# nayuki/DEFLATE-library-Java

Measured on AMD Instinct MI355X. Metric: input MiB/s (compress+decompress), higher is better.
Workload: dtype u8

## Files before the change

### deflate-library-java_amd/csrc/capi/ndfl_deflate_batch_chunked.cpp

```cpp

struct SegTables {
    std::vector<SegChunk> chunks;
    std::vector<SegStream> streams;
    uint64_t staged = 0;
    uint64_t out_bytes = 0;
    bool any_sum = false;
};

static uint64_t seg_out_slot(uint64_t len, uint32_t chunk_len) {
    return ((ndfl_deflate_bound(len, chunk_len) + 8 + 3) / 4 + 2) * 4;
}

static int seg_build_tables(const ndfl_member_item* items, uint32_t n, uint32_t chunk_len, SegTables& T) {
    uint64_t nch = 0;
    for (uint32_t i = 0; i < n; i++) {
        const uint64_t len = items[i].in_len;
        nch += len == 0 ? 1 : len / chunk_len + (len % chunk_len != 0);
        if (nch > 0xFFFFFFFFull) return NDFL_E_UNSUPPORTED;
    }
    T.chunks.resize(nch);
    T.streams.resize(n);
    T.staged = nch * chunk_len;
    T.any_sum = false;
    uint64_t k = 0, obase = 0;
    for (uint32_t i = 0; i < n; i++) {
        const ndfl_member_item& it = items[i];
        const uint64_t len = it.in_len;
        const uint32_t cnt = (uint32_t)(len == 0 ? 1 : len / chunk_len + (len % chunk_len != 0));
        const uint32_t kind = it.format == NDFL_FMT_ZLIB ? NDFL_SUM_ADLER32 : it.format == NDFL_FMT_GZIP ? NDFL_SUM_CRC32 : it.sum;
        T.any_sum = T.any_sum || kind != NDFL_SUM_NONE;
        T.streams[i] = SegStream{obase, (uint32_t)k, cnt};
        obase += seg_out_slot(len, chunk_len);
        for (uint32_t j = 0; j < cnt; j++) {
            const uint64_t at = (uint64_t)j * chunk_len;
            SegChunk& c = T.chunks[k + j];
            c.start = k * chunk_len;
            c.src = it.in_off + at;
            c.stream = i;
            c.len = (uint32_t)std::min<uint64_t>(chunk_len, len - at);
            c.flags = (j == 0 ? SEG_FIRST : 0u) | (j + 1 == cnt ? SEG_LAST : 0u) | kind << SEG_SUM_SHIFT;
            c.pad = 0;
        }
        k += cnt;
    }
    T.out_bytes = obase;
    return NDFL_OK;
}

static int seg_launch_rle(ndfl_ctx* c, hipStream_t s, const SegTab tab, const uint8_t* slots, uint32_t nch, uint64_t staged,
                          uint32_t chunk_len, uint32_t hist_limit, int rle, int dyn) {
    HIPCHK(c->d_hist.ensure((size_t)nch * HREC * 4));
    HIPCHK(c->d_codes.ensure((size_t)nch * CREC * 4));
    const uint32_t ntile = (nch + SCAN_TILE - 1) / SCAN_TILE;
    HIPCHK(c->d_off.ensure(((size_t)2 * nch + 8 + ntile) * 8));
    uint64_t* d_offs = c->d_off.as<uint64_t>();
    uint64_t* d_raw = d_offs + nch;
    uint64_t* d_total = d_raw + nch;
    uint64_t* d_part = d_total + 8;
    Args a;
    a.in = slots; a.n = staged; a.chunk_len = chunk_len; a.nchunks = nch;
    a.prev_byte = -1; a.hist_enabled = hist_limit > 0; a.final_last = 1;
    a.rle = rle; a.dynamic = dyn; a.base_bit = 0; a.parent_len = chunk_len;
    a.out = c->d_out.as<uint32_t>(); a.status = c->d_status.as<uint64_t>(); a.ticket = c->d_ticket.as<uint32_t>();
    a.edge_w = c->d_edge_w.as<uint64_t>(); a.edge_v = c->d_edge_v.as<uint32_t>();
    a.chunk_bits = nullptr; a.crc_raw = nullptr;
    a.crc_tab = c->d_tabs.as<uint32_t>(); a.crc_x = c->d_tabs.as<uint32_t>() + 1024;
    a.prof = nullptr;
    a.hist_out = c->d_hist.as<uint32_t>(); a.codes = c->d_codes.as<uint32_t>(); a.chunk_off = d_offs;
    a.c0 = 0;
    a.pf_dist = c->knobs.deflate_pf ? 2u * (uint32_t)c->ncu : 0u;
    hipLaunchKernelGGL(ndfl_deflate_hist_seg_kernel, dim3(nch), dim3(1024), 0, s, a, tab);
    HIPCHK(hipGetLastError());
    hipLaunchKernelGGL(ndfl_deflate_codes_seg_kernel, dim3(nch), dim3(64), 0, s, a, tab);
    HIPCHK(hipGetLastError());
    hipLaunchKernelGGL(ndfl_deflate_offsets_sum_kernel, dim3(ntile), dim3(SCAN_T), 0, s, (const uint64_t*)a.status, nch, d_part);
    HIPCHK(hipGetLastError());
    hipLaunchKernelGGL(ndfl_deflate_offsets_kernel, dim3(ntile), dim3(SCAN_T), 0, s, (const uint64_t*)a.status, nch,
                       (uint64_t)0, d_raw, d_total, (const uint64_t*)d_part);
    HIPCHK(hipGetLastError());
    hipLaunchKernelGGL(ndfl_deflate_offsets_seg_kernel, dim3((nch + 255) / 256), dim3(256), 0, s, (const uint64_t*)d_raw,
                       a.status, nch, tab, d_offs);
    HIPCHK(hipGetLastError());
    hipLaunchKernelGGL(ndfl_deflate_emit_seg_kernel, dim3(nch), dim3(1024), 0, s, a, tab);
    HIPCHK(hipGetLastError());
    return NDFL_OK;
}

static int seg_launch_lz(ndfl_ctx* c, hipStream_t s, const SegTab tab, const uint8_t* buf, uint32_t nch, uint64_t staged,
                         uint32_t chunk_len, uint32_t hist_limit, const LzTuple& t, int dyn) {
    const uint64_t total = LZ_DS + staged;
    const uint32_t slab_ch = (uint32_t)std::min<uint64_t>(nch, std::max<uint64_t>(1, c->knobs.seg_slab / chunk_len));
    HIPCHK(c->d_match.ensure((size_t)slab_ch * chunk_len * 4));
    LzArgs la;
    la.buf = buf; la.total = total; la.vstart = LZ_DS; la.chunk_len = chunk_len; la.parent_len = chunk_len;
    la.hist_limit = hist_limit; la.min_run = (uint32_t)t.min_run; la.max_run = (uint32_t)t.max_run;
    la.min_dist = (uint32_t)t.min_dist; la.max_dist = (uint32_t)t.max_dist;
    la.link = nullptr; la.L0 = 0; la.match = c->d_match.as<uint32_t>(); la.stats = nullptr;
    LzEncArgs ea;
    ea.match = c->d_match.as<uint32_t>(); ea.n = staged; ea.chunk_len = chunk_len; ea.nchunks = nch;
    ea.final_last = 1; ea.dynamic = dyn; ea.base_bit = 0;
    ea.out = c->d_out.as<uint32_t>(); ea.status = c->d_status.as<uint64_t>(); ea.ticket = c->d_ticket.as<uint32_t>();
    ea.edge_w = c->d_edge_w.as<uint64_t>(); ea.edge_v = c->d_edge_v.as<uint32_t>();
    ea.chunk_bits = nullptr; ea.match_rw = c->d_match.as<uint32_t>();
// ... 33 lines not shown
    SegTab tab;
    tab.chunks = c->d_segtab.as<SegChunk>();
    tab.streams = (const SegStream*)((char*)c->d_segtab.p + chunks_b);

    HIPCHK(c->d_lz.ensure(LZ_DS + T.staged + 64));
    uint8_t* buf = c->d_lz.as<uint8_t>();
    uint8_t* slots = buf + LZ_DS;
    HIPCHK(hipMemsetAsync(buf, 0, LZ_DS, s));
    HIPCHK(hipMemsetAsync(slots + T.staged, 0, 64, s));
    std::unique_ptr<uint8_t[]> pack;
    if (flags & NDFL_IN_DEVICE) {
        hipLaunchKernelGGL(ndfl_seg_gather_kernel, dim3(nch), dim3(256), 0, s, in, slots, tab, chunk_len);
        HIPCHK(hipGetLastError());
    } else {
        pack.reset(new (std::nothrow) uint8_t[T.staged]);
        if (!pack) return NDFL_E_INTERNAL;
        for (uint32_t k = 0; k < nch; k++) {
            const SegChunk& ch = T.chunks[k];
            uint8_t* dst = pack.get() + (uint64_t)k * chunk_len;
            if (ch.len) memcpy(dst, in + ch.src, ch.len);
            if (ch.len < chunk_len) memset(dst + ch.len, 0, chunk_len - ch.len);
        }
        HIPCHK(hipMemcpyAsync(slots, pack.get(), T.staged, hipMemcpyHostToDevice, s));
    }

    HIPCHK(c->d_out.ensure(T.out_bytes));
    HIPCHK(c->d_status.ensure(nch * sizeof(uint64_t)));
    HIPCHK(c->d_ticket.ensure(64));
    HIPCHK(c->d_edge_w.ensure(2ull * nch * sizeof(uint64_t)));
    HIPCHK(c->d_edge_v.ensure(2ull * nch * sizeof(uint32_t)));
    HIPCHK(c->d_crc.ensure(2ull * nch * sizeof(uint32_t)));
    HIPCHK(c->d_crc1.ensure(std::max<size_t>(64, (size_t)n * sizeof(uint32_t))));
    const int preset = lz77_preset(t, dynamic);

    auto launch = [&](hipStream_t q, uint8_t* d_out, const ndfl_member_item* d_items, ndfl_deflate_result* d_res,
                      uint32_t*) -> int {
        HIPCHK(hipMemsetAsync(c->d_status.p, 0, nch * sizeof(uint64_t), q));
        if (preset >= 0)
            TRY(seg_launch_rle(c, q, tab, slots, nch, T.staged, chunk_len, hist_limit,
                               preset == NDFL_RLE_STATIC || preset == NDFL_RLE_DYNAMIC, dynamic != 0));
        else
            TRY(seg_launch_lz(c, q, tab, buf, nch, T.staged, chunk_len, hist_limit, t, dynamic != 0));
        const uint32_t ne = 2 * nch;
        hipLaunchKernelGGL(ndfl_edge_fixup_kernel, dim3((ne + 255) / 256), dim3(256), 0, q, (const uint64_t*)c->d_edge_w.p,
                           (const uint32_t*)c->d_edge_v.p, ne, c->d_out.as<uint32_t>());
        HIPCHK(hipGetLastError());
        uint32_t* d_sums = c->d_crc1.as<uint32_t>();
        if (T.any_sum) {
            hipLaunchKernelGGL(ndfl_seg_sums_kernel, dim3(nch), dim3(1024), 0, q, (const uint8_t*)slots, chunk_len, tab,
                               (const uint32_t*)c->d_tabs.as<uint32_t>(), (const uint32_t*)(c->d_tabs.as<uint32_t>() + 1024),
                               c->d_crc.as<uint32_t>());
            HIPCHK(hipGetLastError());
            hipLaunchKernelGGL(ndfl_seg_sums_combine_kernel, dim3((uint32_t)(((uint64_t)n * 64 + 255) / 256)), dim3(256), 0, q,
                               (const uint32_t*)c->d_crc.p, chunk_len, tab, d_items, n,
                               (const uint32_t*)(c->d_tabs.as<uint32_t>() + 1024 + 64 + 1024), d_sums);
            HIPCHK(hipGetLastError());
        } else {
            HIPCHK(hipMemsetAsync(d_sums, 0, (size_t)n * sizeof(uint32_t), q));
        }
        hipLaunchKernelGGL(ndfl_seg_finish_kernel, dim3(n), dim3(1024), 0, q, c->d_out.as<uint8_t>(),
                           (const uint64_t*)c->d_status.p, tab, d_items, (const uint32_t*)d_sums, d_out, d_res);
        return NDFL_OK;
    };
    return batch_status(batch_run(c->batch, s, c->ev0, c->ev1, out, items, results, n, flags, &c->last_ms, launch));
}

extern "C" int ndfl_deflate_batch_chunked(ndfl_ctx* c, const uint8_t* in, uint64_t in_size, uint8_t* out, uint64_t out_size,
                                          const ndfl_member_item* items, ndfl_deflate_result* results, uint32_t n,
                                          int dynamic, int min_run, int max_run, int min_dist, int max_dist,
                                          uint32_t chunk_len, uint32_t hist_limit, uint32_t flags) {
    if (!c) return NDFL_E_ARG;
    if (n == 0) return NDFL_OK;
    const LzTuple t{min_run, max_run, min_dist, max_dist};
    if (!lz77_tuple_valid(t)) return NDFL_E_ARG;
    if (const int e = deflate_batch_args(in, in_size, out, out_size, items, results, n, chunk_len, hist_limit)) return e;
    return deflate_batch_chunked_run(c, in, out, items, results, n, t, dynamic, chunk_len, hist_limit, flags);
}
```

### deflate-library-java_amd/csrc/capi/ndfl_deflate_chunks.cpp

```cpp
#define TRY(x) do { if (const int _rc = (x)) return _rc; } while (0)

struct LzTuple {
    int min_run, max_run, min_dist, max_dist;
    bool literal_only() const { return min_run == 0 && max_run == 0 && min_dist == 0 && max_dist == 0; }
};
static LzTuple desc_tuple(const ndfl_strategy_desc& d) { return LzTuple{d.min_run, d.max_run, d.min_dist, d.max_dist}; }

static bool lz77_tuple_valid(const LzTuple& t) {
    const int min_run = t.min_run, max_run = t.max_run, min_dist = t.min_dist, max_dist = t.max_dist;
    return t.literal_only() || (3 <= min_run && min_run <= max_run && max_run <= 258 && 1 <= min_dist &&
                                min_dist <= max_dist && max_dist <= 32768);
}

static int lz77_preset(const LzTuple& t, int dynamic) {
    if (t.literal_only()) return dynamic ? NDFL_LITERAL_DYNAMIC : NDFL_LITERAL_STATIC;
    if (t.min_run == 3 && t.max_run == 258 && t.min_dist == 1 && t.max_dist == 1)
        return dynamic ? NDFL_RLE_DYNAMIC : NDFL_RLE_STATIC;
    return -1;
}

struct BlockOpts {
    uint64_t* chunk_bits = nullptr;
    uint32_t parent_len = 0;
};
// ... 106 lines not shown
    HIPCHK(hipMemsetAsync(c->d_ticket.p, 0, 64, s));

    Args a;
    a.in = d_data; a.n = f.len; a.chunk_len = f.chunk_len; a.nchunks = nch;
    a.prev_byte = prev_byte; a.hist_enabled = f.hist_limit > 0; a.final_last = f.final_flag ? 1 : 0;
    a.rle = rle; a.dynamic = dyn; a.base_bit = f.start_bitpos;
    a.parent_len = o.parent_len ? o.parent_len : f.chunk_len;
    a.out = f.d_out; a.status = c->d_status.as<uint64_t>(); a.ticket = c->d_ticket.as<uint32_t>();
    a.edge_w = c->d_edge_w.as<uint64_t>(); a.edge_v = c->d_edge_v.as<uint32_t>();
    a.chunk_bits = o.chunk_bits;
    a.crc_raw = f.crc_inout ? c->d_crc.as<uint32_t>() : nullptr;
    a.crc_tab = c->d_tabs.as<uint32_t>();
    a.crc_x = c->d_tabs.as<uint32_t>() + 1024;
    ScopedBuf prof;
    if (c->knobs.deflate_profile) {
        HIPCHK(prof.ensure((size_t)nch * 64));
        HIPCHK(hipMemsetAsync(prof.p, 0, (size_t)nch * 64, s));
    }
    a.prof = prof.as<uint64_t>();
    a.hist_out = nullptr; a.codes = nullptr; a.chunk_off = nullptr;
    a.pf_dist = c->knobs.deflate_pf ? 2u * (uint32_t)c->ncu : 0u;
    const bool split = !c->knobs.deflate_fused && !prof.p;
    uint64_t* d_total = nullptr;
    if (split) {
        HIPCHK(c->d_hist.ensure((size_t)nch * HREC * 4));
        HIPCHK(c->d_codes.ensure((size_t)nch * CREC * 4));
        HIPCHK(c->d_off.ensure((size_t)nch * 8 + 64 + (size_t)((nch + SCAN_TILE - 1) / SCAN_TILE) * 8));
        a.hist_out = c->d_hist.as<uint32_t>();
        a.codes = c->d_codes.as<uint32_t>();
        a.chunk_off = c->d_off.as<uint64_t>();
        d_total = c->d_off.as<uint64_t>() + nch;
    }
    a.c0 = 0;
    TRY(f.start_timing());
    if (split) {
        hipLaunchKernelGGL(ndfl_deflate_hist_kernel, dim3(nch), dim3(1024), 0, s, a);
        HIPCHK(hipGetLastError());
        hipLaunchKernelGGL(ndfl_deflate_codes_kernel, dim3(nch), dim3(64), 0, s, a);
        HIPCHK(hipGetLastError());
        const uint32_t ntile = (nch + SCAN_TILE - 1) / SCAN_TILE;
        uint64_t* d_part = c->d_off.as<uint64_t>() + nch + 8;
        hipLaunchKernelGGL(ndfl_deflate_offsets_sum_kernel, dim3(ntile), dim3(SCAN_T), 0, s, (const uint64_t*)a.status,
                           nch, d_part);
        HIPCHK(hipGetLastError());
        hipLaunchKernelGGL(ndfl_deflate_offsets_kernel, dim3(ntile), dim3(SCAN_T), 0, s, (const uint64_t*)a.status, nch,
                           (uint64_t)f.start_bitpos, c->d_off.as<uint64_t>(), d_total, (const uint64_t*)d_part);
        HIPCHK(hipGetLastError());
        hipLaunchKernelGGL(ndfl_deflate_emit_kernel, dim3(nch), dim3(1024), 0, s, a);
    } else {
        hipLaunchKernelGGL(ndfl_deflate_chunks_kernel, dim3(nch), dim3(1024), 0, s, a);
    }
    HIPCHK(hipGetLastError());
    TRY(f.stop_timing());
    const uint32_t ne = 2 * nch;
    hipLaunchKernelGGL(ndfl_edge_fixup_kernel, dim3((ne + 255) / 256), dim3(256), 0, s,
                       (const uint64_t*)a.edge_w, (const uint32_t*)a.edge_v, ne, f.d_out);
    HIPCHK(hipGetLastError());
    if (f.crc_inout) {
        HIPCHK(launch_crc_combine(c, s, (const uint32_t*)a.crc_raw, nch, f.chunk_len, f.len, c->d_crc1.as<uint32_t>()));
        HIPCHK(hipMemcpyAsync(c->h_pinned + 4, c->d_crc1.p, 4, hipMemcpyDeviceToHost, s));
    }
    TRY(f.read_end(split ? d_total : a.status + (nch - 1)));
    if (prof.p) {
        std::vector<uint64_t> h((size_t)nch * 8);
        HIPCHK(hipMemcpy(h.data(), prof.p, (size_t)nch * 64, hipMemcpyDeviceToHost));
        double sum[7] = {0}, tmin = 1e300, tmax = 0;
        for (uint32_t k = 0; k < nch; k++) {
            const uint64_t* q = &h[k * 8];
            for (int p = 0; p < 7; p++) sum[p] += (double)(q[p + 1] - q[p]);
            tmin = std::min(tmin, (double)q[0]); tmax = std::max(tmax, (double)q[7]);
        }
        fprintf(stderr, "[ndfl] deflate phases (us/chunk): load+crc %.2f hist %.2f codes %.2f bits+scan %.2f emit %.2f "
                "lookback %.2f store %.2f; span %.2f ms\n", sum[0] / nch / 100, sum[1] / nch / 100, sum[2] / nch / 100,
                sum[3] / nch / 100, sum[4] / nch / 100, sum[5] / nch / 100, sum[6] / nch / 100, (tmax - tmin) / 1e5);
    }
    if (f.crc_inout) {
        uint32_t raw = c->h_pinned[4];
        uint32_t dc = ~(crc_multmodp(crc_x8n(f.len), 0xFFFFFFFFu) ^ raw);
        *f.crc_inout = ndfl_crc32_combine(*f.crc_inout, dc, f.len);
    }
    return f.finish();
}

static int chunks_lz(Frame& f, const LzTuple& t, int dyn, BlockOpts o) {
    ndfl_ctx* c = f.c;
    hipStream_t s = f.s;
    const uint32_t nch = f.nch, chunk_len = f.chunk_len;
    const uint64_t len = f.len;
    const uint64_t total = LZ_DS + len;
    HIPCHK(c->d_lz.ensure(total + 64));
    uint8_t* buf = c->d_lz.as<uint8_t>();
    const hipMemcpyKind kin = (f.flags & NDFL_IN_DEVICE) ? hipMemcpyDeviceToDevice : hipMemcpyHostToDevice;
    if (f.hist_len) HIPCHK(hipMemcpyAsync(buf + LZ_DS - f.hist_len, f.hist, f.hist_len, kin, s));
    if (len) HIPCHK(hipMemcpyAsync(buf + LZ_DS, f.data, len, kin, s));
    HIPCHK(hipMemsetAsync(buf + total, 0, 64, s));
// ... 408 lines not shown
```

### deflate-library-java_amd/csrc/hip/deflate_kernels.hip

```cpp
#pragma once
#include "huffman_build.hpp"
#include "seg_tables.hpp"

namespace {

constexpr int DT = 1024;
constexpr int NW = DT / 64;
constexpr int MAX_CHUNK = 65536;
constexpr int OUTW = 18600;
static_assert(sizeof(HuffScr) <= OUTW * 4, "the code-construction scratch is laid over the bit buffer");

constexpr uint64_t ST_AGG = 1ull << 62;
constexpr uint64_t ST_PRE = 2ull << 62;
constexpr uint64_t ST_VAL = (1ull << 62) - 1;

struct Persist {
    uint32_t litCode[288];
    uint32_t distCode[32];
    uint64_t scan64[NW];
    uint32_t scan32[NW];
    uint32_t chunk;
    uint32_t hdrBits;
    uint64_t P;
    uint32_t crcAcc[NW];
};

struct Args {
    const uint8_t* in;
    uint64_t n;
    uint32_t chunk_len;
    uint32_t nchunks;
    int32_t prev_byte;
    int32_t hist_enabled;
    int32_t final_last;
    int32_t rle;
    int32_t dynamic;
    uint32_t parent_len;
    uint32_t base_bit;
    uint32_t* out;
    uint64_t* status;
    uint32_t* ticket;
    uint64_t* edge_w;
    uint32_t* edge_v;
    uint64_t* chunk_bits;
    uint32_t* crc_raw;
    const uint32_t* crc_tab;
    const uint32_t* crc_x;
    uint64_t* prof;
    uint32_t* hist_out;
    const uint32_t* codes;
    const uint64_t* chunk_off;
    uint32_t c0;
    uint32_t pf_dist;
};

constexpr int HREC = 320;
constexpr int CREC_LIT = 0;
constexpr int CREC_DIST = 288;
constexpr int CREC_HDR = 320;
constexpr int CREC_META = CREC_HDR + HDRW;
constexpr int CREC = CREC_META + 16;
enum { MODE_FUSED = 0, MODE_HIST = 1, MODE_EMIT = 2 };
#ifndef NDFL_HCOPY
#define NDFL_HCOPY 8
#endif
constexpr int HCOPY = NDFL_HCOPY;
constexpr int HSTR = HCOPY > 4 ? 340 : 336;

__device__ __forceinline__ void run_sym(uint32_t run, uint32_t& sym, uint32_t& ne, uint32_t& ex) {
    if (run < 11) { sym = run + 254; ne = 0; ex = 0; }
    else if (run == 258) { sym = 285; ne = 0; ex = 0; }
    else {
        uint32_t r = run - 3;
        ne = 29 - __builtin_clz(r);
        sym = (ne << 2) + (r >> ne) + 257;
        ex = r & ((1u << ne) - 1);
    }
}

template <bool SEG = false>
__device__ __forceinline__ void block_lookback(uint32_t c, uint64_t base_bit, uint64_t S, uint64_t* status, Persist& ps,
                                               bool first = false) {
    const int tid = threadIdx.x;
    const int lane = tid & 63, wid = tid >> 6;
    if (wid == 0) {
        uint64_t P = base_bit;
// ... 45 lines not shown
    be.put(code & 0xFFFF, code >> 16);
    be.flush();
}

}

template <int MODE, bool SEG = false>
__device__ __forceinline__ void deflate_chunk(const Args& a, uint32_t* obuf, Persist& ps, uint32_t* hdrw = nullptr,
                                              uint32_t* hl4 = nullptr, uint32_t* ctab = nullptr, const SegTab t = SegTab{}) {
    static_assert(!SEG || MODE != MODE_FUSED, "the one-kernel encoder is not segmented");
    HuffScr* scr = (HuffScr*)obuf;
    uint32_t* hlit = scr->hlit;
    uint32_t* hdist = scr->hdist;
    uint8_t* lastb = MODE == MODE_HIST ? (uint8_t*)obuf : scr->lastb;

    const int tid = threadIdx.x;
    const int lane = tid & 63, wid = tid >> 6;

    const uint64_t tp0 = wall_clock64();
    if (MODE == MODE_FUSED) {
        if (tid == 0) ps.chunk = atomicAdd(a.ticket, 1u);
    } else {
        if (tid == 0) ps.chunk = a.c0 + blockIdx.x;
    }
    if (MODE == MODE_FUSED) {
        if (tid < 288) hlit[tid] = 0;
        if (tid < 32) hdist[tid] = 0;
    } else if (MODE == MODE_HIST) {
        for (int k = tid; k < HCOPY * HSTR; k += DT) hl4[k] = 0;
        if (a.crc_raw) ctab[tid] = a.crc_tab[tid];
    }
    __syncthreads();
    uint32_t c = ps.chunk;
    if constexpr (SEG) c = a.c0 + blockIdx.x;
    const uint64_t cs = (uint64_t)c * a.chunk_len;
    uint32_t segf = 0;
    if constexpr (SEG) segf = t.chunks[c].flags;
    const uint32_t len_c = SEG ? t.chunks[c].len : (uint32_t)min((uint64_t)a.chunk_len, a.n - cs);
    const bool is_final = SEG ? (segf & SEG_LAST) != 0 : a.final_last && (c + 1 == a.nchunks);
    const bool first = SEG && (segf & SEG_FIRST) != 0;
    const uint8_t* src = a.in + cs;

    uint32_t w[16];
    const uint32_t t0 = (uint32_t)tid * 64;
    const int vcnt = (int)min(64u, len_c > t0 ? len_c - t0 : 0u);
    if (vcnt == 64 && (((uintptr_t)(src + t0)) & 15) == 0) {
        const u32x4* p = (const u32x4*)(src + t0);
#pragma unroll
        for (int k = 0; k < 4; k++) {
            u32x4 v = __builtin_nontemporal_load(p + k);
            w[4 * k] = v.x; w[4 * k + 1] = v.y; w[4 * k + 2] = v.z; w[4 * k + 3] = v.w;
        }
    } else {
#pragma unroll
        for (int k = 0; k < 16; k++) {
            uint32_t x = 0;
#pragma unroll
            for (int b = 0; b < 4; b++) {
                int i = 4 * k + b;
                if (i < vcnt) x |= (uint32_t)src[t0 + i] << (8 * b);
            }
            w[k] = x;
        }
    }
    if (vcnt > 0) {
        uint32_t lv = w[15] >> 24;
        if (vcnt < 64) {
// ... 81 lines not shown
    uint32_t mpx = 0xFFFFu;
    if (vcnt > 0) {
        mpx = nextStart - t0;
        if (a.rle && tid == 0 && (F & 1) && lead_of(0, w[0] & 0xFFu) == 0) mpx |= 1u << 31;
    }
    uint64_t LM = 0, LG = 0;
    uint32_t ce = 0;
    if (vcnt > 0) {
        const uint32_t mq = mpx & 0xFFFFu;
        const uint64_t wl = F | (mq < 64 ? 1ull << mq : 0ull);
        const uint64_t wh = (mq >= 64 && mq < 67) ? 1ull << (mq - 64) : 0ull;
        const uint64_t e1 = (wl >> 1) | (wh << 63), e2 = (wl >> 2) | (wh << 62), e3 = (wl >> 3) | (wh << 61);
        uint64_t r3 = F & ~e1 & ~e2 & e3;
        LG = F & ~(e1 | e2 | e3);
        if ((mpx >> 31) && (r3 & 1ull)) { r3 &= ~1ull; LG |= 1ull; }
        const uint64_t r2 = (F & ~e1 & e2) | r3;
        const uint64_t r1 = (F & e1) | r2;
        LM = r1 | (r2 << 1) | (r3 << 2);
        ce = (uint32_t)(r2 >> 63) + (uint32_t)((r3 >> 62) & 1ull) + (uint32_t)(r3 >> 63);
    }
#define NDFL_FOR_GROUPS_L(...)                                                                         \
    _Pragma("unroll 1") for (int o_ = 0; o_ < 8; o_++) {                                               \
        const uint32_t lm_ = (uint32_t)(LM >> (8 * o_)) & 0xFFu;                                      \
        const uint32_t lg_ = (uint32_t)(LG >> (8 * o_)) & 0xFFu;                                      \
        if (!__any((lm_ | lg_) != 0)) continue;                                                        \
        const bool o1_ = o_ & 1, o2_ = o_ & 2, o4_ = o_ & 4;                                           \
        const uint32_t a0_ = o1_ ? w[2] : w[0], a1_ = o1_ ? w[6] : w[4];                               \
        const uint32_t a2_ = o1_ ? w[10] : w[8], a3_ = o1_ ? w[14] : w[12];                            \
        const uint32_t b0_ = o1_ ? w[3] : w[1], b1_ = o1_ ? w[7] : w[5];                               \
        const uint32_t b2_ = o1_ ? w[11] : w[9], b3_ = o1_ ? w[15] : w[13];                            \
        const uint32_t gw0_ = o4_ ? (o2_ ? a3_ : a2_) : (o2_ ? a1_ : a0_);                             \
        const uint32_t gw1_ = o4_ ? (o2_ ? b3_ : b2_) : (o2_ ? b1_ : b0_);                             \
        const bool anyL_ = __any(lg_ != 0);                                                            \
        __VA_ARGS__                                                                                    \
    }
#define NDFL_BYTE(j) ((((j) < 4 ? gw0_ : gw1_) >> (8 * ((j) & 3))) & 0xFFu)
#define NDFL_LMASK(j) ((uint32_t)((int32_t)(lm_ << (31 - (j))) >> 31))
#define NDFL_RUN_L(j, ...)                                                                             \
    if ((lg_ >> (j)) & 1) {                                                                            \
        const int i_ = 8 * o_ + (j);                                                                   \
        const uint32_t v = NDFL_BYTE(j);                                                               \
        const uint32_t gpos = t0 + (uint32_t)i_;                                                       \
        const uint64_t rest_ = i_ < 63 ? (F >> (i_ + 1)) : 0ull;                                       \
        const uint32_t pend = rest_ ? gpos + 1 + (uint32_t)__builtin_ctzll(rest_) : nextStart;         \
        __VA_ARGS__                                                                                    \
    }

    uint32_t* hl = hlit;
    uint32_t* hd = hdist;
    if (MODE == MODE_HIST) { hl = hl4 + (tid & (HCOPY - 1)) * HSTR; hd = hl + 288; }
    if (MODE == MODE_HIST) {
        asm volatile("" :: "v"(prev0));
        prefetch_next();
    }
    if (MODE != MODE_EMIT) {
    NDFL_FOR_GROUPS_L({
_Pragma("unroll")
        for (int j = 0; j < 8; j++)
            if ((lm_ >> j) & 1) atomicAdd(&hl[NDFL_BYTE(j)], 1u);
        if (!anyL_) continue;
_Pragma("unroll")
        for (int j = 0; j < 8; j++) {
            NDFL_RUN_L(j, {
                const uint32_t lead = lead_of(gpos, v);
                const uint32_t R = pend - gpos - lead;
                const uint32_t n258 = R / 258, m = R % 258;
                const uint32_t nlit = lead + (m < 3 ? m : 0);
                if (nlit) atomicAdd(&hl[v], nlit);
                if (n258) atomicAdd(&hl[285], n258);
                uint32_t nd = n258;
                if (m >= 3) {
                    uint32_t sym, ne, ex; run_sym(m, sym, ne, ex);
                    atomicAdd(&hl[sym], 1u);
                    nd++;
                }
// ... 7 lines not shown
        if (a.dynamic && len_c == 0) atomicAdd(&hl[0], 1u);
    }
    __syncthreads();
    }
    if (MODE == MODE_HIST) {
        uint32_t* h = a.hist_out + (uint64_t)c * HREC;
        if (tid < HREC) {
            uint32_t v = 0;
_Pragma("unroll")
            for (int k = 0; k < HCOPY; k++) v += hl4[k * HSTR + tid];
            h[tid] = v;
        }
        asm volatile("" :: "v"(pfv));
        return;
    }

    const uint64_t tp2 = wall_clock64();
    if constexpr (MODE == MODE_FUSED) {
        const uint32_t hb = build_block_codes<DT>(*scr, a.dynamic != 0, is_final, ps.litCode, ps.distCode);
        if (tid < HDRW) hdrw[tid] = scr->hdr()[tid];
        if (tid == 0) ps.hdrBits = hb;
    } else {
        const uint32_t* rec = a.codes + (uint64_t)c * CREC;
        if (tid < 288) ps.litCode[tid] = rec[CREC_LIT + tid];
        else if (tid < 320) ps.distCode[tid - 288] = rec[CREC_DIST + tid - 288];
        if (tid == 0) ps.hdrBits = rec[CREC_META];
    }
    __syncthreads();

    const uint64_t tp3 = wall_clock64();
    if (MODE == MODE_EMIT) prefetch_next();
    const uint32_t d0 = __builtin_amdgcn_readfirstlane(ps.distCode[0]);
    const uint32_t c285 = __builtin_amdgcn_readfirstlane(ps.litCode[285]);
    uint32_t mybits = 0;
    NDFL_FOR_GROUPS_L({
        uint32_t pf[8];
_Pragma("unroll")
        for (int j = 0; j < 8; j++) pf[j] = ps.litCode[NDFL_BYTE(j)];
        uint32_t gs = 0;
_Pragma("unroll")
        for (int j = 0; j < 8; j++) gs += (pf[j] & NDFL_LMASK(j)) >> 16;
        mybits += gs;
        if (anyL_) {
_Pragma("unroll")
            for (int j = 0; j < 8; j++) {
                NDFL_RUN_L(j, {
                    const uint32_t lv = pf[j] >> 16;
                    const uint32_t lead = lead_of(gpos, v);
                    const uint32_t R = pend - gpos - lead;
                    const uint32_t n258 = R / 258, m = R % 258;
                    mybits += lead * lv + n258 * ((c285 >> 16) + (d0 >> 16));
                    if (m >= 3) {
                        uint32_t sym, ne, ex; run_sym(m, sym, ne, ex);
                        mybits += (ps.litCode[sym] >> 16) + ne + (d0 >> 16);
                    } else {
                        mybits += m * lv;
                    }
                })
            }
        }
    })
    if (ce) mybits += ce * (ps.litCode[w[15] >> 24] >> 16);
    const uint64_t tp3a = wall_clock64();
    uint32_t tokTotal;
    const uint32_t myoff = block_excl_scan<uint32_t, NW>(mybits, ps.scan32, tokTotal);
    const uint64_t tp3b = wall_clock64();
    const uint32_t eobLen = __builtin_amdgcn_readfirstlane(ps.litCode[256] >> 16);
    const uint32_t hdrBits = __builtin_amdgcn_readfirstlane(ps.hdrBits);
    const uint64_t S = (uint64_t)hdrBits + tokTotal + eobLen;
    if (MODE == MODE_FUSED && tid == 0) {
        if (c == 0) st_agent(&a.status[0], ST_PRE | (a.base_bit + S));
        else st_agent(&a.status[c], ST_AGG | S);
        if (a.chunk_bits) a.chunk_bits[c] = S;
    }
    const uint64_t tp4 = wall_clock64();
    const uint32_t nwl = (uint32_t)((S + 31) >> 5) + 1;
    __syncthreads();
    {
        const uint32_t* hdr = MODE == MODE_FUSED ? hdrw : a.codes + (uint64_t)c * CREC + CREC_HDR;
        const uint32_t hw = (hdrBits + 31) >> 5;
        for (uint32_t k = (uint32_t)tid; k < nwl; k += DT) obuf[k] = k < hw ? hdr[k] : 0u;
    }
    __syncthreads();
    const uint32_t bit0 = 0;

    if (tid == 0) put_end_of_block(obuf, bit0 + hdrBits + tokTotal, ps.litCode[256]);
    {
        BitPut bp; bp.init(obuf, bit0 + hdrBits + myoff);
        const uint32_t d0c = d0 & 0xFFFF, d0l = d0 >> 16;
        const uint32_t m258 = (c285 & 0xFFFF) | (d0c << (c285 >> 16));
        const uint32_t m258l = (c285 >> 16) + d0l;
        NDFL_FOR_GROUPS_L({
            uint32_t pf[4];
_Pragma("unroll")
            for (int j = 0; j < 4; j++) pf[j] = ps.litCode[NDFL_BYTE(j)];
            if (!anyL_) {
_Pragma("unroll")
                for (int j = 0; j < 8; j += 2) {
                    const uint32_t e0 = pf[j & 3] & NDFL_LMASK(j);
                    const uint32_t e1 = pf[(j + 1) & 3] & NDFL_LMASK(j + 1);
                    if (j < 4) { pf[j] = ps.litCode[NDFL_BYTE(j + 4)]; pf[j + 1] = ps.litCode[NDFL_BYTE(j + 5)]; }
                    const uint32_t l0 = e0 >> 16;
                    bp.put((e0 & 0xFFFF) | ((e1 & 0xFFFF) << l0), l0 + (e1 >> 16));
                }
                continue;
            }
_Pragma("unroll")
            for (int j = 0; j < 8; j++) {
                const uint32_t lc = pf[j & 3];
                if (j < 4) pf[j] = ps.litCode[NDFL_BYTE(j + 4)];
                const uint32_t e = lc & NDFL_LMASK(j);
                bp.put(e & 0xFFFF, e >> 16);
                NDFL_RUN_L(j, {
                    const uint32_t lead = lead_of(gpos, v);
                    const uint32_t R = pend - gpos - lead;
                    const uint32_t n258 = R / 258, m = R % 258;
                    if (lead) bp.put(lc & 0xFFFF, lc >> 16);
                    for (uint32_t k = 0; k < n258; k++) bp.put(m258, m258l);
                    if (m >= 3) {
                        uint32_t sym, ne, ex; run_sym(m, sym, ne, ex);
                        const uint32_t sc = ps.litCode[sym];
                        bp.put(sc & 0xFFFF, sc >> 16);
                        bp.put(ex, ne);
                        bp.put(d0c, d0l);
                    } else {
                        for (uint32_t k = 0; k < m; k++) bp.put(lc & 0xFFFF, lc >> 16);
                    }
                })
            }
        })
        if (ce) {
            const uint32_t lc = ps.litCode[w[15] >> 24];
            bp.put(lc & 0xFFFF, lc >> 16);
            if (ce > 1) bp.put(lc & 0xFFFF, lc >> 16);
        }
        bp.flush();
    }
    __syncthreads();

    const uint64_t tp5e = wall_clock64();
    if constexpr (MODE == MODE_FUSED) block_lookback(c, a.base_bit, S, a.status, ps);
    const uint64_t tp5 = wall_clock64();
    const uint64_t P = MODE == MODE_FUSED ? ps.P : a.chunk_off[c];
    block_store(obuf, P, S, c, a.out, a.edge_w, a.edge_v);
    if (tid == 0) {
        if (a.prof) {
            uint64_t* q = a.prof + (uint64_t)c * 8;
            q[0] = tp0; q[1] = tp1; q[2] = tp2; q[3] = tp3; q[4] = tp4; q[5] = tp5e; q[6] = tp5;
            q[7] = wall_clock64();
            (void)tp3a; (void)tp3b;
        }
    }
    (void)is_final; (void)first;
    asm volatile("" :: "v"(pfv));
}

extern "C" __global__ void __launch_bounds__(DT, 8)
ndfl_deflate_chunks_kernel(Args a) {
    __shared__ __attribute__((aligned(16))) uint32_t obuf[OUTW];
    __shared__ Persist ps;
    __shared__ uint32_t hdrw[HDRW];
    deflate_chunk<MODE_FUSED>(a, obuf, ps, hdrw);
}

extern "C" __global__ void __launch_bounds__(DT, 8)
ndfl_deflate_hist_kernel(Args a) {
    __shared__ __attribute__((aligned(16))) uint32_t lastb[1024 / 4];
    __shared__ __attribute__((aligned(16))) uint32_t hl4[HCOPY * HSTR];
    __shared__ uint32_t ctab[1024];
    __shared__ Persist ps;
    deflate_chunk<MODE_HIST>(a, lastb, ps, nullptr, hl4, ctab);
}
extern "C" __global__ void __launch_bounds__(DT, 8)
ndfl_deflate_hist_seg_kernel(Args a, SegTab t) {
    __shared__ __attribute__((aligned(16))) uint32_t lastb[1024 / 4];
    __shared__ __attribute__((aligned(16))) uint32_t hl4[HCOPY * HSTR];
    __shared__ uint32_t ctab[1024];
    __shared__ Persist ps;
    deflate_chunk<MODE_HIST, true>(a, lastb, ps, nullptr, hl4, ctab, t);
}

extern "C" __global__ void __launch_bounds__(DT, 8)
ndfl_deflate_emit_kernel(Args a) {
    __shared__ __attribute__((aligned(16))) uint32_t obuf[OUTW];
    __shared__ Persist ps;
    deflate_chunk<MODE_EMIT>(a, obuf, ps);
}
extern "C" __global__ void __launch_bounds__(DT, 8)
ndfl_deflate_emit_seg_kernel(Args a, SegTab t) {
    __shared__ __attribute__((aligned(16))) uint32_t obuf[OUTW];
    __shared__ Persist ps;
    deflate_chunk<MODE_EMIT, true>(a, obuf, ps, nullptr, nullptr, nullptr, t);
}

extern "C" __global__ void ndfl_edge_fixup_kernel(const uint64_t* edge_w, const uint32_t* edge_v, uint32_t n_edges,
                                                  uint32_t* out) {
    uint32_t e = blockIdx.x * blockDim.x + threadIdx.x;
    if (e >= n_edges) return;
    uint64_t wv = edge_w[e];
    if (e > 0 && edge_w[e - 1] == wv) return;
    uint32_t v = 0;
    for (uint32_t k = e; k < n_edges && edge_w[k] == wv; k++) v |= edge_v[k];
    out[wv] = v;
}

extern "C" __global__ void __launch_bounds__(256)
ndfl_crc_combine_kernel(const uint32_t* crc_raw, uint32_t nchunks, uint32_t chunk_len, uint64_t n,
                        const uint32_t* x8p2, uint32_t* out_raw) {
    uint32_t acc = 0;
    for (uint32_t c = blockIdx.x * blockDim.x + threadIdx.x; c < nchunks; c += gridDim.x * blockDim.x) {
        const uint64_t end = min((uint64_t)(c + 1) * chunk_len, n);
        uint64_t after = n - end;
        uint32_t p = 1u << 31;
        for (int k = 0; after; k++, after >>= 1)
            if (after & 1) p = crc_multmodp(x8p2[k], p);
        acc ^= crc_multmodp(p, crc_raw[c]);
    }
    acc = wave_xor(acc);
    if ((threadIdx.x & 63) == 0 && acc) atomicXor(out_raw, acc);
// ... 84 lines not shown
```

### deflate-library-java_amd/csrc/hip/huffman_build.hpp

```cpp
#pragma once
#include "ndfl_common.hpp"

namespace {

constexpr int HDRW = 80;

struct BitPut {
    uint32_t lo;
    uint32_t nb;
    uint32_t wb;
    char* buf;
    __device__ __forceinline__ void init(uint32_t* b, uint32_t bitpos) {
        buf = (char*)b; wb = (bitpos >> 5) * 4; nb = bitpos & 31; lo = 0;
    }
    __device__ __forceinline__ void put(uint32_t v, uint32_t n) {
        const uint32_t nb0 = nb;
        lo |= v << nb0;
        nb = nb0 + n;
        if (nb >= 32) {
            atomicOr((uint32_t*)(buf + wb), lo);
            wb += 4;
            nb -= 32;
            lo = v >> (32 - nb0);
        }
    }
    __device__ __forceinline__ void flush() {
        if (nb) atomicOr((uint32_t*)(buf + wb), lo);
    }
};

constexpr uint32_t CL_EXTRA_BITS[3] = {2, 3, 7};
constexpr uint8_t CL_ORDER[19] = {16, 17, 18, 0, 8, 7, 9, 6, 10, 5, 11, 4, 12, 3, 13, 2, 14, 1, 15};

struct HuffScr {
    uint32_t hlit[288];
    uint32_t hdist[32];
    uint32_t hdist0[32];
    union {
        uint32_t lf[288];
        uint16_t clOff[320];
    };
    uint16_t ls[288];
    union {
        uint32_t pf[2][304];
        uint8_t lastb[1024];
    };
    __device__ __forceinline__ uint32_t* key() { return pf[1]; }
    __device__ __forceinline__ uint32_t* hdr() { return pf[0]; }
    uint32_t mpk[15 * 20];
    uint32_t lvl[16];
    __device__ __forceinline__ uint32_t* scan() { return lvl; }
    uint32_t blc[16], nxc[16], mask[16 * 10];
    uint32_t clh[20];
    uint32_t clCode[20];
    uint32_t misc[8];
    uint8_t clSym[320], clExtra[320];
    uint8_t lens[320];
    uint8_t clLen[32];
};

template <bool OPQ>
// ... 321 lines not shown
```

### deflate-library-java_amd/csrc/hip/ndfl_common.hpp

```cpp
#pragma once
#include <hip/hip_runtime.h>
#include <stdint.h>
#include <stdio.h>
#include <stdlib.h>
#include <string.h>

struct Knobs {
    bool stats = false;
    bool host_times = false;
    bool host_link = false;
    bool no_hdrrec = false;
    bool emit_fast = true;
    bool no_bt = false;
    bool no_alias = false;
    uint32_t count_w = 0;
    bool deflate_pf = true;
    bool deflate_profile = false;
    bool deflate_fused = false;
    bool lz_stats = false;
    bool lz_chain = false;
    int lz_lead = -1;
    bool flat = true;
    uint32_t flat_min = 49152;
    bool test_segflip = false;
    uint32_t batch_waves = 0;
    uint64_t seg_slab = 256ull << 20;
    void read() {
        auto on = [](const char* n) { const char* e = getenv(n); return e && strcmp(e, "0") != 0; };
        auto num = [](const char* n, int dflt) { const char* e = getenv(n); return e ? atoi(e) : dflt; };
        stats = on("NDFL_STATS"); host_times = on("NDFL_HOST_TIMES"); host_link = on("NDFL_HOST_LINK");
        no_hdrrec = on("NDFL_NO_HDRREC");
        emit_fast = num("NDFL_EMIT_FAST", 1) != 0;
        no_bt = on("NDFL_NO_BT"); no_alias = on("NDFL_NO_ALIAS");
        count_w = (uint32_t)num("NDFL_COUNT_W", 0);
        deflate_pf = num("NDFL_DEFLATE_PF", 1) != 0; deflate_profile = on("NDFL_DEFLATE_PROFILE");
        deflate_fused = on("NDFL_DEFLATE_FUSED");
        lz_stats = on("NDFL_LZ_STATS");
        const char* se = getenv("NDFL_LZ_SEARCH");
        lz_chain = se && !strcmp(se, "chain");
        lz_lead = num("NDFL_LZ_LEAD", -1);
        test_segflip = on("NDFL_TEST_SEGFLIP");
        flat = num("NDFL_FLAT", 1) != 0;
        flat_min = (uint32_t)num("NDFL_FLAT_MIN", 49152);
        { const int bw = num("NDFL_BATCH_WAVES", 0); batch_waves = bw > 0 ? (uint32_t)bw : 0u; }
        { const char* e = getenv("NDFL_SEG_SLAB"); const long long v = e ? atoll(e) : 0; if (v > 0) seg_slab = (uint64_t)v; }
    }
    void print(FILE* f) const {
        fprintf(f, "[ndfl] context knobs: stats=%d host_times=%d host_link=%d no_hdrrec=%d emit_fast=%d no_bt=%d "
                   "no_alias=%d count_w=%u deflate_pf=%d deflate_profile=%d deflate_fused=%d lz_stats=%d "
                   "lz_search=%s lz_lead=%d test_segflip=%d flat=%d flat_min=%u batch_waves=%u seg_slab=%llu\n",
                (int)stats, (int)host_times, (int)host_link, (int)no_hdrrec, (int)emit_fast, (int)no_bt,
                (int)no_alias, count_w, (int)deflate_pf, (int)deflate_profile, (int)deflate_fused, (int)lz_stats,
                lz_chain ? "chain" : "parse", lz_lead, (int)test_segflip, (int)flat, flat_min, batch_waves,
                (unsigned long long)seg_slab);
    }
};

#define NDFL_WAVE 64

typedef uint32_t u32x4 __attribute__((ext_vector_type(4)));

#define NDFL_CRC_POLY 0xEDB88320u

__host__ __device__ inline uint32_t crc_multmodp(uint32_t a, uint32_t b) {
    uint32_t m = 1u << 31, p = 0;
    for (;;) {
        if (a & m) {
            p ^= b;
            if ((a & (m - 1)) == 0) break;
        }
        m >>= 1;
        b = (b & 1) ? (b >> 1) ^ NDFL_CRC_POLY : b >> 1;
    }
    return p;
}

__host__ __device__ inline uint32_t crc_x8n(uint64_t n) {
    uint32_t p = 1u << 31;
    uint32_t sq = 1u << 23;
    while (n) {
        if (n & 1) p = crc_multmodp(sq, p);
        sq = crc_multmodp(sq, sq);
        n >>= 1;
    }
    return p;
// ... 147 lines not shown
```

Baseline: 212,800.

## Emit deflate tokens in a single walk via per-lane LDS slots

```diff
diff --git a/deflate-library-java_amd/csrc/capi/ndfl_deflate_batch_chunked.cpp b/deflate-library-java_amd/csrc/capi/ndfl_deflate_batch_chunked.cpp
--- a/deflate-library-java_amd/csrc/capi/ndfl_deflate_batch_chunked.cpp
+++ b/deflate-library-java_amd/csrc/capi/ndfl_deflate_batch_chunked.cpp
@@ -48,7 +48,7 @@
 }
 
 static int seg_launch_rle(ndfl_ctx* c, hipStream_t s, const SegTab tab, const uint8_t* slots, uint32_t nch, uint64_t staged,
-                          uint32_t chunk_len, uint32_t hist_limit, int rle, int dyn) {
+                          uint32_t chunk_len, uint32_t hist_limit, int rle, int dyn, uint32_t* two_walks) {
     HIPCHK(c->d_hist.ensure((size_t)nch * HREC * 4));
     HIPCHK(c->d_codes.ensure((size_t)nch * CREC * 4));
     const uint32_t ntile = (nch + SCAN_TILE - 1) / SCAN_TILE;
@@ -69,6 +69,8 @@
     a.hist_out = c->d_hist.as<uint32_t>(); a.codes = c->d_codes.as<uint32_t>(); a.chunk_off = d_offs;
     a.c0 = 0;
     a.pf_dist = c->knobs.deflate_pf ? 2u * (uint32_t)c->ncu : 0u;
+    a.onewalk = c->knobs.deflate_onewalk ? 1u : 0u;
+    a.two_walks = two_walks;
     hipLaunchKernelGGL(ndfl_deflate_hist_seg_kernel, dim3(nch), dim3(1024), 0, s, a, tab);
     HIPCHK(hipGetLastError());
     hipLaunchKernelGGL(ndfl_deflate_codes_seg_kernel, dim3(nch), dim3(64), 0, s, a, tab);
@@ -168,13 +170,17 @@
     HIPCHK(c->d_crc.ensure(2ull * nch * sizeof(uint32_t)));
     HIPCHK(c->d_crc1.ensure(std::max<size_t>(64, (size_t)n * sizeof(uint32_t))));
     const int preset = lz77_preset(t, dynamic);
+    ScopedBuf two_walks;
+    if (c->knobs.stats && preset >= 0) HIPCHK(two_walks.ensure(64));
 
     auto launch = [&](hipStream_t q, uint8_t* d_out, const ndfl_member_item* d_items, ndfl_deflate_result* d_res,
                       uint32_t*) -> int {
         HIPCHK(hipMemsetAsync(c->d_status.p, 0, nch * sizeof(uint64_t), q));
+        if (two_walks.p) HIPCHK(hipMemsetAsync(two_walks.p, 0, 64, q));
         if (preset >= 0)
             TRY(seg_launch_rle(c, q, tab, slots, nch, T.staged, chunk_len, hist_limit,
-                               preset == NDFL_RLE_STATIC || preset == NDFL_RLE_DYNAMIC, dynamic != 0));
+                               preset == NDFL_RLE_STATIC || preset == NDFL_RLE_DYNAMIC, dynamic != 0,
+                               two_walks.as<uint32_t>()));
         else
             TRY(seg_launch_lz(c, q, tab, buf, nch, T.staged, chunk_len, hist_limit, t, dynamic != 0));
         const uint32_t ne = 2 * nch;
@@ -198,7 +204,13 @@
                            (const uint64_t*)c->d_status.p, tab, d_items, (const uint32_t*)d_sums, d_out, d_res);
         return NDFL_OK;
     };
-    return batch_status(batch_run(c->batch, s, c->ev0, c->ev1, out, items, results, n, flags, &c->last_ms, launch));
+    const int rc = batch_status(batch_run(c->batch, s, c->ev0, c->ev1, out, items, results, n, flags, &c->last_ms, launch));
+    if (two_walks.p && rc == NDFL_OK) {
+        uint32_t tw = 0;
+        HIPCHK(hipMemcpy(&tw, two_walks.p, 4, hipMemcpyDeviceToHost));
+        fprintf(stderr, "[ndfl] deflate emit: %u chunks, %u took two walks\n", nch, tw);
+    }
+    return rc;
 }
 
 extern "C" int ndfl_deflate_batch_chunked(ndfl_ctx* c, const uint8_t* in, uint64_t in_size, uint8_t* out, uint64_t out_size,
diff --git a/deflate-library-java_amd/csrc/capi/ndfl_deflate_chunks.cpp b/deflate-library-java_amd/csrc/capi/ndfl_deflate_chunks.cpp
--- a/deflate-library-java_amd/csrc/capi/ndfl_deflate_chunks.cpp
+++ b/deflate-library-java_amd/csrc/capi/ndfl_deflate_chunks.cpp
@@ -162,6 +162,13 @@
         d_total = c->d_off.as<uint64_t>() + nch;
     }
     a.c0 = 0;
+    a.onewalk = c->knobs.deflate_onewalk ? 1u : 0u;
+    ScopedBuf two_walks;
+    if (c->knobs.stats && split) {
+        HIPCHK(two_walks.ensure(64));
+        HIPCHK(hipMemsetAsync(two_walks.p, 0, 64, s));
+    }
+    a.two_walks = two_walks.as<uint32_t>();
     TRY(f.start_timing());
     if (split) {
         hipLaunchKernelGGL(ndfl_deflate_hist_kernel, dim3(nch), dim3(1024), 0, s, a);
@@ -191,6 +198,11 @@
         HIPCHK(hipMemcpyAsync(c->h_pinned + 4, c->d_crc1.p, 4, hipMemcpyDeviceToHost, s));
     }
     TRY(f.read_end(split ? d_total : a.status + (nch - 1)));
+    if (two_walks.p) {
+        uint32_t tw = 0;
+        HIPCHK(hipMemcpy(&tw, two_walks.p, 4, hipMemcpyDeviceToHost));
+        fprintf(stderr, "[ndfl] deflate emit: %u chunks, %u took two walks\n", nch, tw);
+    }
     if (prof.p) {
         std::vector<uint64_t> h((size_t)nch * 8);
         HIPCHK(hipMemcpy(h.data(), prof.p, (size_t)nch * 64, hipMemcpyDeviceToHost));
diff --git a/deflate-library-java_amd/csrc/hip/deflate_kernels.hip b/deflate-library-java_amd/csrc/hip/deflate_kernels.hip
--- a/deflate-library-java_amd/csrc/hip/deflate_kernels.hip
+++ b/deflate-library-java_amd/csrc/hip/deflate_kernels.hip
@@ -9,6 +9,12 @@
 constexpr int MAX_CHUNK = 65536;
 constexpr int OUTW = 18600;
 static_assert(sizeof(HuffScr) <= OUTW * 4, "the code-construction scratch is laid over the bit buffer");
+constexpr uint32_t SLOTW = 18;
+using SlotPut = BitPutSlot<SLOTW, DT>;
+constexpr uint32_t SLOT_OVER = 1u << 20;
+static_assert(DT * SLOTW <= OUTW, "the lanes' slots are laid over the bit buffer");
+static_assert(OUTW * 32 < SLOT_OVER && (uint64_t)DT * SLOT_OVER + OUTW * 32 < (1ull << 32),
+              "a chunk's token bits and the count of lanes past their slots share one 32-bit sum");
 
 constexpr uint64_t ST_AGG = 1ull << 62;
 constexpr uint64_t ST_PRE = 2ull << 62;
@@ -52,6 +58,8 @@
     const uint64_t* chunk_off;
     uint32_t c0;
     uint32_t pf_dist;
+    uint32_t onewalk;
+    uint32_t* two_walks;
 };
 
 constexpr int HREC = 320;
@@ -163,7 +171,7 @@
     }
     __syncthreads();
     uint32_t c = ps.chunk;
-    if constexpr (SEG) c = a.c0 + blockIdx.x;
+    if constexpr (SEG || MODE == MODE_EMIT) c = a.c0 + blockIdx.x;
     const uint64_t cs = (uint64_t)c * a.chunk_len;
     uint32_t segf = 0;
     if constexpr (SEG) segf = t.chunks[c].flags;
@@ -311,6 +319,8 @@
         const uint32_t gw0_ = o4_ ? (o2_ ? a3_ : a2_) : (o2_ ? a1_ : a0_);                             \
         const uint32_t gw1_ = o4_ ? (o2_ ? b3_ : b2_) : (o2_ ? b1_ : b0_);                             \
         const bool anyL_ = __any(lg_ != 0);                                                            \
+        uint32_t gb_ = 0;                                                                              \
+        if (MODE == MODE_EMIT) { gb_ = t0 + 8u * (uint32_t)o_; asm volatile("" : "+v"(gb_)); }         \
         __VA_ARGS__                                                                                    \
     }
 #define NDFL_BYTE(j) ((((j) < 4 ? gw0_ : gw1_) >> (8 * ((j) & 3))) & 0xFFu)
@@ -319,7 +329,7 @@
     if ((lg_ >> (j)) & 1) {                                                                            \
         const int i_ = 8 * o_ + (j);                                                                   \
         const uint32_t v = NDFL_BYTE(j);                                                               \
-        const uint32_t gpos = t0 + (uint32_t)i_;                                                       \
+        const uint32_t gpos = MODE == MODE_EMIT ? gb_ + (j) : t0 + (uint32_t)i_;                       \
         const uint64_t rest_ = i_ < 63 ? (F >> (i_ + 1)) : 0ull;                                       \
         const uint32_t pend = rest_ ? gpos + 1 + (uint32_t)__builtin_ctzll(rest_) : nextStart;         \
         __VA_ARGS__                                                                                    \
@@ -393,7 +403,71 @@
     if (MODE == MODE_EMIT) prefetch_next();
     const uint32_t d0 = __builtin_amdgcn_readfirstlane(ps.distCode[0]);
     const uint32_t c285 = __builtin_amdgcn_readfirstlane(ps.litCode[285]);
-    uint32_t mybits = 0;
+    const uint32_t d0c = d0 & 0xFFFF, d0l = d0 >> 16;
+    const uint32_t m258 = (c285 & 0xFFFF) | (d0c << (c285 >> 16));
+    const uint32_t m258l = (c285 >> 16) + d0l;
+#define NDFL_TOKEN_WALK(BP)                                                                            \
+    NDFL_FOR_GROUPS_L({                                                                                \
+        uint32_t pf[4];                                                                                \
+_Pragma("unroll")                                                                                      \
+        for (int j = 0; j < 4; j++) pf[j] = ps.litCode[NDFL_BYTE(j)];                                  \
+        if (!anyL_) {                                                                                  \
+_Pragma("unroll")                                                                                      \
+            for (int j = 0; j < 8; j += 2) {                                                           \
+                const uint32_t e0 = pf[j & 3] & NDFL_LMASK(j);                                         \
+                const uint32_t e1 = pf[(j + 1) & 3] & NDFL_LMASK(j + 1);                               \
+                if (j < 4) { pf[j] = ps.litCode[NDFL_BYTE(j + 4)]; pf[j + 1] = ps.litCode[NDFL_BYTE(j + 5)]; } \
+                const uint32_t l0 = e0 >> 16;                                                          \
+                BP.put((e0 & 0xFFFF) | ((e1 & 0xFFFF) << l0), l0 + (e1 >> 16));                        \
+            }                                                                                          \
+            continue;                                                                                  \
+        }                                                                                              \
+_Pragma("unroll")                                                                                      \
+        for (int j = 0; j < 8; j++) {                                                                  \
+            const uint32_t lc = pf[j & 3];                                                             \
+            if (j < 4) pf[j] = ps.litCode[NDFL_BYTE(j + 4)];                                           \
+            const uint32_t e = lc & NDFL_LMASK(j);                                                     \
+            BP.put(e & 0xFFFF, e >> 16);                                                               \
+            NDFL_RUN_L(j, {                                                                            \
+                const uint32_t lead = lead_of(gpos, v);                                                \
+                const uint32_t R = pend - gpos - lead;                                                 \
+                const uint32_t n258 = R / 258, m = R % 258;                                            \
+                if (lead) BP.put(lc & 0xFFFF, lc >> 16);                                               \
+                for (uint32_t k = 0; k < n258; k++) BP.put(m258, m258l);                               \
+                if (m >= 3) {                                                                          \
+                    uint32_t sym, ne, ex; run_sym(m, sym, ne, ex);                                     \
+                    const uint32_t sc = ps.litCode[sym];                                               \
+                    BP.put(sc & 0xFFFF, sc >> 16);                                                     \
+                    BP.put(ex, ne);                                                                    \
+                    BP.put(d0c, d0l);                                                                  \
+                } else {                                                                               \
+                    for (uint32_t k = 0; k < m; k++) BP.put(lc & 0xFFFF, lc >> 16);                    \
+                }                                                                                      \
+            })                                                                                         \
+        }                                                                                              \
+    })                                                                                                 \
+    if (ce) {                                       \
+        const uint32_t lc = ps.litCode[w[15] >> 24];                                                   \
+        BP.put(lc & 0xFFFF, lc >> 16);                                                                 \
+        if (ce > 1) BP.put(lc & 0xFFFF, lc >> 16);                                                     \
+    }                                                                                                  \
+    BP.flush();
+    bool onewalk = false;
+    uint32_t mybits = 0, myoff = 0, tokTotal = 0;
+    if constexpr (MODE == MODE_EMIT) {
+        if (a.onewalk) {
+            SlotPut bs; bs.init(obuf);
+            NDFL_TOKEN_WALK(bs)
+            mybits = bs.bits();
+            myoff = block_excl_scan<uint32_t, NW>(mybits + (mybits > SLOTW * 32 ? SLOT_OVER : 0u), ps.scan32, tokTotal);
+            tokTotal = __builtin_amdgcn_readfirstlane(tokTotal);
+            onewalk = tokTotal < SLOT_OVER;
+        }
+        if (!onewalk && tid == 0 && a.two_walks) atomicAdd(a.two_walks, 1u);
+    }
+    const uint64_t tp3a = wall_clock64();
+    if (!onewalk) {
+    mybits = 0;
     NDFL_FOR_GROUPS_L({
         uint32_t pf[8];
 _Pragma("unroll")
@@ -422,9 +496,8 @@
         }
     })
     if (ce) mybits += ce * (ps.litCode[w[15] >> 24] >> 16);
-    const uint64_t tp3a = wall_clock64();
-    uint32_t tokTotal;
-    const uint32_t myoff = block_excl_scan<uint32_t, NW>(mybits, ps.scan32, tokTotal);
+    myoff = block_excl_scan<uint32_t, NW>(mybits, ps.scan32, tokTotal);
+    }
     const uint64_t tp3b = wall_clock64();
     const uint32_t eobLen = __builtin_amdgcn_readfirstlane(ps.litCode[256] >> 16);
     const uint32_t hdrBits = __builtin_amdgcn_readfirstlane(ps.hdrBits);
@@ -436,66 +509,40 @@
     }
     const uint64_t tp4 = wall_clock64();
     const uint32_t nwl = (uint32_t)((S + 31) >> 5) + 1;
-    __syncthreads();
-    {
+    auto zero_buffer = [&]() {
         const uint32_t* hdr = MODE == MODE_FUSED ? hdrw : a.codes + (uint64_t)c * CREC + CREC_HDR;
         const uint32_t hw = (hdrBits + 31) >> 5;
         for (uint32_t k = (uint32_t)tid; k < nwl; k += DT) obuf[k] = k < hw ? hdr[k] : 0u;
-    }
-    __syncthreads();
+    };
     const uint32_t bit0 = 0;
 
-    if (tid == 0) put_end_of_block(obuf, bit0 + hdrBits + tokTotal, ps.litCode[256]);
-    {
+    if (MODE == MODE_EMIT && onewalk) {
+        const uint32_t nsw = (mybits + 31) >> 5;
+        uint32_t sw[SLOTW];
+#pragma unroll
+        for (uint32_t k = 0; k < SLOTW; k++) sw[k] = k < nsw ? obuf[SlotPut::word(k)] : 0u;
+        __syncthreads();
+        zero_buffer();
+        __syncthreads();
+        if (tid == 0) put_end_of_block(obuf, bit0 + hdrBits + tokTotal, ps.litCode[256]);
+        const uint32_t B = bit0 + hdrBits + myoff;
+        const uint32_t sh = B & 31;
+        uint32_t* dst = obuf + (B >> 5);
+        const uint32_t ndw = mybits ? (sh + mybits + 31) >> 5 : 0u;
+#pragma unroll
+        for (uint32_t k = 0; k <= SLOTW; k++) {
+            const uint32_t cur = k < SLOTW ? sw[k] : 0u;
+            const uint32_t prv = k ? sw[k - 1] : 0u;
+            const uint32_t v = sh ? (cur << sh) | (prv >> (32 - sh)) : cur;
+            if (k < ndw) atomicOr(&dst[k], v);
+        }
+    } else {
+        __syncthreads();
+        zero_buffer();
+        __syncthreads();
+        if (tid == 0) put_end_of_block(obuf, bit0 + hdrBits + tokTotal, ps.litCode[256]);
         BitPut bp; bp.init(obuf, bit0 + hdrBits + myoff);
-        const uint32_t d0c = d0 & 0xFFFF, d0l = d0 >> 16;
-        const uint32_t m258 = (c285 & 0xFFFF) | (d0c << (c285 >> 16));
-        const uint32_t m258l = (c285 >> 16) + d0l;
-        NDFL_FOR_GROUPS_L({
-            uint32_t pf[4];
-_Pragma("unroll")
-            for (int j = 0; j < 4; j++) pf[j] = ps.litCode[NDFL_BYTE(j)];
-            if (!anyL_) {
-_Pragma("unroll")
-                for (int j = 0; j < 8; j += 2) {
-                    const uint32_t e0 = pf[j & 3] & NDFL_LMASK(j);
-                    const uint32_t e1 = pf[(j + 1) & 3] & NDFL_LMASK(j + 1);
-                    if (j < 4) { pf[j] = ps.litCode[NDFL_BYTE(j + 4)]; pf[j + 1] = ps.litCode[NDFL_BYTE(j + 5)]; }
-                    const uint32_t l0 = e0 >> 16;
-                    bp.put((e0 & 0xFFFF) | ((e1 & 0xFFFF) << l0), l0 + (e1 >> 16));
-                }
-                continue;
-            }
-_Pragma("unroll")
-            for (int j = 0; j < 8; j++) {
-                const uint32_t lc = pf[j & 3];
-                if (j < 4) pf[j] = ps.litCode[NDFL_BYTE(j + 4)];
-                const uint32_t e = lc & NDFL_LMASK(j);
-                bp.put(e & 0xFFFF, e >> 16);
-                NDFL_RUN_L(j, {
-                    const uint32_t lead = lead_of(gpos, v);
-                    const uint32_t R = pend - gpos - lead;
-                    const uint32_t n258 = R / 258, m = R % 258;
-                    if (lead) bp.put(lc & 0xFFFF, lc >> 16);
-                    for (uint32_t k = 0; k < n258; k++) bp.put(m258, m258l);
-                    if (m >= 3) {
-                        uint32_t sym, ne, ex; run_sym(m, sym, ne, ex);
-                        const uint32_t sc = ps.litCode[sym];
-                        bp.put(sc & 0xFFFF, sc >> 16);
-                        bp.put(ex, ne);
-                        bp.put(d0c, d0l);
-                    } else {
-                        for (uint32_t k = 0; k < m; k++) bp.put(lc & 0xFFFF, lc >> 16);
-                    }
-                })
-            }
-        })
-        if (ce) {
-            const uint32_t lc = ps.litCode[w[15] >> 24];
-            bp.put(lc & 0xFFFF, lc >> 16);
-            if (ce > 1) bp.put(lc & 0xFFFF, lc >> 16);
-        }
-        bp.flush();
+        NDFL_TOKEN_WALK(bp)
     }
     __syncthreads();
 
@@ -546,6 +593,7 @@
     __shared__ __attribute__((aligned(16))) uint32_t obuf[OUTW];
     __shared__ Persist ps;
     deflate_chunk<MODE_EMIT>(a, obuf, ps);
+    asm volatile("" ::: "v63");
 }
 extern "C" __global__ void __launch_bounds__(DT, 8)
 ndfl_deflate_emit_seg_kernel(Args a, SegTab t) {
diff --git a/deflate-library-java_amd/csrc/hip/huffman_build.hpp b/deflate-library-java_amd/csrc/hip/huffman_build.hpp
--- a/deflate-library-java_amd/csrc/hip/huffman_build.hpp
+++ b/deflate-library-java_amd/csrc/hip/huffman_build.hpp
@@ -27,6 +27,32 @@
     __device__ __forceinline__ void flush() {
         if (nb) atomicOr((uint32_t*)(buf + wb), lo);
     }
+};
+
+template <uint32_t SLOTW, uint32_t NT>
+struct BitPutSlot {
+    static_assert((NT & (NT - 1)) == 0, "a power of two");
+    uint32_t lo;
+    uint32_t nb;
+    uint32_t wb;
+    char* buf;
+    static __device__ __forceinline__ uint32_t word(uint32_t k) { return k * NT + threadIdx.x; }
+    __device__ __forceinline__ void init(uint32_t* b) { buf = (char*)b; wb = threadIdx.x * 4; nb = 0; lo = 0; }
+    __device__ __forceinline__ void put(uint32_t v, uint32_t n) {
+        const uint32_t nb0 = nb;
+        lo |= v << nb0;
+        nb = nb0 + n;
+        if (nb >= 32) {
+            if (wb < SLOTW * NT * 4) *(uint32_t*)(buf + wb) = lo;
+            wb += NT * 4;
+            nb -= 32;
+            lo = v >> (32 - nb0);
+        }
+    }
+    __device__ __forceinline__ void flush() {
+        if (nb && wb < SLOTW * NT * 4) *(uint32_t*)(buf + wb) = lo;
+    }
+    __device__ __forceinline__ uint32_t bits() const { return wb / (NT * 4) * 32 + nb; }
 };
 
 constexpr uint32_t CL_EXTRA_BITS[3] = {2, 3, 7};
diff --git a/deflate-library-java_amd/csrc/hip/ndfl_common.hpp b/deflate-library-java_amd/csrc/hip/ndfl_common.hpp
--- a/deflate-library-java_amd/csrc/hip/ndfl_common.hpp
+++ b/deflate-library-java_amd/csrc/hip/ndfl_common.hpp
@@ -17,6 +17,7 @@
     bool deflate_pf = true;
     bool deflate_profile = false;
     bool deflate_fused = false;
+    bool deflate_onewalk = true;
     bool lz_stats = false;
     bool lz_chain = false;
     int lz_lead = -1;
@@ -35,6 +36,7 @@
         count_w = (uint32_t)num("NDFL_COUNT_W", 0);
         deflate_pf = num("NDFL_DEFLATE_PF", 1) != 0; deflate_profile = on("NDFL_DEFLATE_PROFILE");
         deflate_fused = on("NDFL_DEFLATE_FUSED");
+        deflate_onewalk = num("NDFL_DEFLATE_ONEWALK", 1) != 0;
         lz_stats = on("NDFL_LZ_STATS");
         const char* se = getenv("NDFL_LZ_SEARCH");
         lz_chain = se && !strcmp(se, "chain");
@@ -47,10 +49,11 @@
     }
     void print(FILE* f) const {
         fprintf(f, "[ndfl] context knobs: stats=%d host_times=%d host_link=%d no_hdrrec=%d emit_fast=%d no_bt=%d "
-                   "no_alias=%d count_w=%u deflate_pf=%d deflate_profile=%d deflate_fused=%d lz_stats=%d "
+                   "no_alias=%d count_w=%u deflate_pf=%d deflate_profile=%d deflate_fused=%d deflate_onewalk=%d lz_stats=%d "
                    "lz_search=%s lz_lead=%d test_segflip=%d flat=%d flat_min=%u batch_waves=%u seg_slab=%llu\n",
                 (int)stats, (int)host_times, (int)host_link, (int)no_hdrrec, (int)emit_fast, (int)no_bt,
-                (int)no_alias, count_w, (int)deflate_pf, (int)deflate_profile, (int)deflate_fused, (int)lz_stats,
+                (int)no_alias, count_w, (int)deflate_pf, (int)deflate_profile, (int)deflate_fused,
+                (int)deflate_onewalk, (int)lz_stats,
                 lz_chain ? "chain" : "parse", lz_lead, (int)test_segflip, (int)flat, flat_min, batch_waves,
                 (unsigned long long)seg_slab);
     }
```

After: 218,400 (median of 6 runs). 1.03x the previous value.
